# santiagolmedo/gnn_qot_estimation

Measured on NVIDIA B200. Metric: lightpath_infer_graphs_per_sec, higher is better.
Workload: dtype f32

## Files before the change

### gnn_qot_estimation_b200/csrc/lightpath_stream.cu

```cuda
#include <algorithm>
#include <type_traits>

#include "lightpath_common.cuh"

namespace qot {

constexpr int kTG = 16;
constexpr int kTNodes = 704;
constexpr int kTEdges = 2688;
constexpr int kTMaxE = 248;
#ifndef QOT_ST_WARPS
#define QOT_ST_WARPS 15
#endif
#ifndef QOT_ST_XSTAGES
#define QOT_ST_XSTAGES 7
#endif
#ifndef QOT_ST_DSTAGES
#define QOT_ST_DSTAGES 4
#endif
#ifndef QOT_STH_WARPS
#define QOT_STH_WARPS 14
#endif
#ifndef QOT_STH_XSTAGES
#define QOT_STH_XSTAGES 6
#endif
#ifndef QOT_STH_DSTAGES
#define QOT_STH_DSTAGES 3
#endif
template <bool kHead> struct StCfg;
template <> struct StCfg<false> {
  static constexpr int kX = QOT_ST_XSTAGES;
  static constexpr int kD = QOT_ST_DSTAGES;
  static constexpr int kConsumers = QOT_ST_WARPS;
  static constexpr int kThreads = 32 * (1 + kConsumers);
};
template <> struct StCfg<true> {
  static constexpr int kX = QOT_STH_XSTAGES;
  static constexpr int kD = QOT_STH_DSTAGES;
  static constexpr int kConsumers = QOT_STH_WARPS;
  static constexpr int kThreads = 32 * (8 + kConsumers - 2);
};
constexpr int kStGroupWarps = 4;
constexpr int kStXBytes = kTNodes * kF * 4;
constexpr int kStDBytes = kTEdges * 8;

struct alignas(16) StTileInfo {
  qot_lp_batch_t d;
  int64_t g0;
  int64_t nb0, eb0;
  int xn, en;
  unsigned xlead, dlead;
  int ng;
  int pad;
};
static_assert(sizeof(qot_lp_batch_t) == 128, "the descriptor is copied as eight 16-byte pieces");

struct alignas(128) StStage {
  alignas(128) unsigned char xs[kStXBytes + 16];
  alignas(16) long long ptrs[3][kTG + 2];
  StTileInfo info;
};
struct alignas(128) StDStage {
  alignas(128) unsigned char ds[kStDBytes + 16];
};

struct StGenericArgs {
  const float* x;
  const int64_t* esrc;
  const int64_t* edst;
  float* z;
  float* out;
  int64_t* lut_batch;
  int32_t* lut_node;
  int32_t* status;
  int64_t N, E, g0;
  int64_t p[4][6];
};

struct StWarpScratch {
  StGenericArgs gargs;
  int msg[4][kSubMsg];
  int raw[4][kSubMsg];
};

constexpr int kZPitch = 21;
constexpr int kGroupTiles = 8;
struct StHeadSmem {
  alignas(1024) float b2[2][4][32 * 32];
  float zrow[2][128 * kZPitch];
  float* optr[2][128];
  alignas(8) unsigned long long zfull[2];
  alignas(8) unsigned long long zfree[2];
  alignas(8) unsigned long long aready;
  alignas(8) unsigned long long dready;
  unsigned tmem_base;
  alignas(16) float wf[kHC * kF];
  alignas(16) float shift[kHC];
  alignas(16) float b1[kHid];
  alignas(16) float w2[QOT_OUT * kHid];
  float bo[4];
};
struct StNoHead {};

template <bool kHead>
struct StSmemT {
  typename std::conditional<kHead, StHeadSmem, StNoHead>::type head;
  StDStage dstage[StCfg<kHead>::kD];
  StStage stage[StCfg<kHead>::kX];
  float4 asp[8][6];
  float4 adp[4][kF];
  StWarpScratch wsc[StCfg<kHead>::kConsumers];
  float gen[256];
  alignas(8) unsigned long long full[StCfg<kHead>::kX];
  alignas(8) unsigned long long empty[StCfg<kHead>::kX];
  alignas(8) unsigned long long dempty[StCfg<kHead>::kD];
  int next_unit;
  int gen_lock;
};
extern __shared__ __align__(1024) char st_smem_raw[];
template <bool kHead>
__device__ __forceinline__ StSmemT<kHead>& st_smem() {
  const unsigned off = (1024u - (static_cast<unsigned>(__cvta_generic_to_shared(st_smem_raw)) & 1023u)) & 1023u;
  return *reinterpret_cast<StSmemT<kHead>*>(st_smem_raw + off);
}
static_assert(sizeof(StSmemT<false>) + 1024 <= 227 * 1024, "lp_stream_kernel: shared memory over the 227 KB block limit");
static_assert(sizeof(StSmemT<true>) + 1024 <= 227 * 1024, "lp_stream_kernel<head>: shared memory over the 227 KB block limit");

#ifdef QOT_ST_TRACE
__device__ unsigned long long* g_st_trace = nullptr;
#define ST_DECL() long long st_acc_[8] = {0, 0, 0, 0, 0, 0, 0, 0}
#define ST_T0() const long long st_t0_ = clock64()
#define ST_T1() const long long st_t1_ = clock64()
#define ST_PARAM , long long* st_acc_
#define ST_ARG , st_acc_
#define ST_ACC1(slot) do { st_acc_[slot] += clock64() - st_t1_; } while (0)
#define ST_ACC(slot) do { st_acc_[slot] += clock64() - st_t0_; } while (0)
#define ST_FLUSH() do { if (g_st_trace && lane == 0) for (int i_ = 0; i_ < 8; ++i_) if (st_acc_[i_]) atomicAdd(g_st_trace + blockIdx.x * 8 + i_, static_cast<unsigned long long>(st_acc_[i_])); } while (0)
#else
#define ST_DECL() do {} while (0)
#define ST_T0() do {} while (0)
#define ST_T1() do {} while (0)
#define ST_PARAM
#define ST_ARG
#define ST_ACC1(slot) do {} while (0)
#define ST_ACC(slot) do {} while (0)
#define ST_FLUSH() do {} while (0)
#endif
__device__ __forceinline__ unsigned st_smem_u32(const void* p) { return static_cast<unsigned>(__cvta_generic_to_shared(p)); }
#ifndef QOT_ST_SUSPEND_NS
#define QOT_ST_SUSPEND_NS 20000
#endif
__device__ __forceinline__ bool st_try_wait(unsigned bar, unsigned parity) {
  unsigned ok;
  asm volatile(
      "{ .reg .pred p; mbarrier.try_wait.parity.shared::cta.b64 p, [%1], %2, %3; selp.u32 %0, 1, 0, p; }"
      : "=r"(ok) : "r"(bar), "r"(parity), "r"(QOT_ST_SUSPEND_NS) : "memory");
  return ok != 0u;
}
template <unsigned kSleepNs = 40>
__device__ __forceinline__ bool st_wait(unsigned bar, unsigned parity) {
  if (st_try_wait(bar, parity)) return true;
  unsigned long long t0;
  asm volatile("mov.u64 %0, %%globaltimer;" : "=l"(t0));
  for (;;) {
#pragma unroll 1
    for (int i = 0; i < 256; ++i) {
      __nanosleep(kSleepNs);
      if (st_try_wait(bar, parity)) return true;
    }
    unsigned long long t1;
    asm volatile("mov.u64 %0, %%globaltimer;" : "=l"(t1));
    if (t1 - t0 > 2000000000ull) return false;
  }
}
__device__ __forceinline__ void st_arrive(unsigned bar) {
  asm volatile("mbarrier.arrive.shared::cta.b64 _, [%0];" ::"r"(bar) : "memory");
}
__device__ __forceinline__ void st_mbar_init(unsigned long long* bar, int count) {
  asm volatile("mbarrier.init.shared::cta.b64 [%0], %1;" ::"r"(st_smem_u32(bar)), "r"(count) : "memory");
}

template <bool kHead>
__device__ __noinline__ void st_producer(const qot_lp_batch_t* __restrict__ bt, int nb, int64_t tpb,
                                         int64_t tile_base, int64_t total_tiles, int lane) {
  StSmemT<kHead>& sm = st_smem<kHead>();
  const int64_t G = gridDim.x;
  const int64_t my_tiles = (total_tiles - blockIdx.x + G - 1) / G;
  ST_DECL();
  for (int64_t kb = 0; kb < my_tiles; kb += 32) {
    int b = 0;
    long long g0 = 0, nb0 = 0, nb1 = 0, eb0 = 0, eb1 = 0, dN = 0, dE = 0, dB = 0;
    const float* dx = nullptr;
    const int64_t *dei = nullptr, *dptr = nullptr, *deptr = nullptr, *dlptr = nullptr;
    if (kb + lane < my_tiles) {
      const int64_t T = tile_base + blockIdx.x + (kb + lane) * G;
      b = st_batch_of(bt, nb, tpb, tile_base, T);
      const qot_lp_batch_t& d = bt[b];
      dx = d.x; dei = d.edge_index; dptr = d.ptr; deptr = d.edge_ptr; dlptr = d.lut_ptr;
      dN = d.N; dE = d.E; dB = d.B;
      g0 = (T - d.tile0) * kTG;
      const int64_t gE = min(static_cast<int64_t>(g0 + kTG), static_cast<int64_t>(dB));
      nb0 = dptr[g0]; nb1 = dptr[gE];
      eb0 = deptr[g0]; eb1 = deptr[gE];
    }
    const int cnt = static_cast<int>(min(static_cast<int64_t>(32), my_tiles - kb));
    for (int j = 0; j < cnt; ++j) {
      const int64_t k = kb + j;
      constexpr int kStStages = StCfg<kHead>::kX, kStDStages = StCfg<kHead>::kD;
      const int s = static_cast<int>(k % kStStages);
      const unsigned ph = static_cast<unsigned>((k / kStStages) & 1);
      StStage& st = sm.stage[s];
      const int sd_ = static_cast<int>(k % kStDStages);
      StDStage& dst_stage = sm.dstage[sd_];
      const unsigned fbar = st_smem_u32(&sm.full[s]);
      {
        ST_T0();
        st_wait(st_smem_u32(&sm.empty[s]), ph ^ 1u);
        st_wait(st_smem_u32(&sm.dempty[sd_]), static_cast<unsigned>((k / kStDStages) & 1) ^ 1u);
        ST_ACC(0);
      }
      ST_T0();
      const int tb = __shfl_sync(kFull, b, j);
      const long long tg0 = __shfl_sync(kFull, g0, j), tB = __shfl_sync(kFull, dB, j);
      const int64_t* tptr = reinterpret_cast<const int64_t*>(__shfl_sync(kFull, reinterpret_cast<unsigned long long>(dptr), j));
      const int64_t* teptr = reinterpret_cast<const int64_t*>(__shfl_sync(kFull, reinterpret_cast<unsigned long long>(deptr), j));
      const int64_t* tlptr = reinterpret_cast<const int64_t*>(__shfl_sync(kFull, reinterpret_cast<unsigned long long>(dlptr), j));
#pragma unroll
      for (int r = 0; r < 2; ++r) {
        const int idx = lane + 32 * r;
        if (idx < 3 * (kTG + 1)) {
          const int which = idx / (kTG + 1), i = idx % (kTG + 1);
          const int64_t gi = min(static_cast<int64_t>(tg0 + i), static_cast<int64_t>(tB));
          const int64_t* src = (which == 0 ? tptr : which == 1 ? teptr : tlptr) + gi;
          asm volatile("cp.async.ca.shared.global [%0], [%1], 8;" ::"r"(st_smem_u32(&st.ptrs[which][i])), "l"(src) : "memory");
        }
      }
      if (lane >= 24)
        asm volatile("cp.async.cg.shared.global [%0], [%1], 16;"
                     ::"r"(st_smem_u32(reinterpret_cast<char*>(&st.info.d) + 16 * (lane - 24))),
                       "l"(reinterpret_cast<const char*>(bt + tb) + 16 * (lane - 24)) : "memory");
      asm volatile("cp.async.mbarrier.arrive.noinc.shared::cta.b64 [%0];" ::"r"(fbar) : "memory");
      if (lane == j) {
        int xn = 0, en = 0;
        if (nb0 >= 0 && nb1 >= nb0 && nb1 <= dN && nb1 - nb0 <= kTNodes) xn = static_cast<int>(nb1 - nb0);
        if (eb0 >= 0 && eb1 >= eb0 && eb1 <= dE && eb1 - eb0 <= kTEdges) en = static_cast<int>(eb1 - eb0);
        if (xn == 0 || (en == 0 && eb1 != eb0)) { xn = 0; en = 0; }
        const int64_t* edst = dei + dE;
        const uintptr_t xa = reinterpret_cast<uintptr_t>(dx) + static_cast<uintptr_t>(xn > 0 ? nb0 : 0) * (kF * 4);
        const uintptr_t da = reinterpret_cast<uintptr_t>(edst) + static_cast<uintptr_t>(en > 0 ? eb0 : 0) * 8;
        const unsigned xlead = static_cast<unsigned>(xa & 15), dlead = static_cast<unsigned>(da & 15);
        const uintptr_t xs0 = xa - xlead, ds0 = da - dlead;
        const unsigned xspan = xlead + static_cast<unsigned>(xn) * (kF * 4), dspan = dlead + static_cast<unsigned>(en) * 8;
        unsigned xbytes = (xspan + 15u) & ~15u, dbytes = (dspan + 15u) & ~15u;
        if (xs0 + xbytes > reinterpret_cast<uintptr_t>(dx) + static_cast<uintptr_t>(dN) * (kF * 4)) xbytes = xspan & ~15u;
        if (ds0 + dbytes > reinterpret_cast<uintptr_t>(edst) + static_cast<uintptr_t>(dE) * 8) dbytes = dspan & ~15u;
        if (xn == 0) xbytes = 0;
        if (en == 0) dbytes = 0;
        if (xn > 0)
          for (unsigned o = xbytes; o < xspan; o += 4)
            *reinterpret_cast<float*>(st.xs + o) = *reinterpret_cast<const float*>(xs0 + o);
        if (en > 0 && dspan > dbytes)
          *reinterpret_cast<long long*>(dst_stage.ds + dbytes) = *reinterpret_cast<const long long*>(ds0 + dbytes);
        StTileInfo& ti = st.info;
        ti.g0 = g0; ti.nb0 = nb0; ti.eb0 = eb0;
        ti.xn = xn; ti.en = en; ti.xlead = xlead; ti.dlead = dlead;
        ti.ng = static_cast<int>(min(static_cast<int64_t>(kTG), static_cast<int64_t>(dB - g0)));
        asm volatile("mbarrier.arrive.expect_tx.shared::cta.b64 _, [%0], %1;" ::"r"(fbar), "r"(xbytes + dbytes) : "memory");
        if (xbytes)
          asm volatile("cp.async.bulk.shared::cluster.global.mbarrier::complete_tx::bytes [%0], [%1], %2, [%3];"
                       ::"r"(st_smem_u32(st.xs)), "l"(xs0), "r"(xbytes), "r"(fbar) : "memory");
        if (dbytes)
          asm volatile("cp.async.bulk.shared::cluster.global.mbarrier::complete_tx::bytes [%0], [%1], %2, [%3];"
                       ::"r"(st_smem_u32(dst_stage.ds)), "l"(ds0), "r"(dbytes), "r"(fbar) : "memory");
      }
      __syncwarp();
      ST_ACC(1);
    }
  }
  ST_FLUSH();
}

template <bool kHead>
__device__ __noinline__ void st_generic(int cw, unsigned todo, const float* __restrict__ prep, int lut_col, int lane) {
  StSmemT<kHead>& sm = st_smem<kHead>();
  const StGenericArgs& ga = sm.wsc[cw].gargs;
  float* scratch = sm.gen;
  int* lock = &sm.gen_lock;
  const float* gx = ga.x;
  const int64_t N = ga.N;
  if (lane == 0)
    while (atomicCAS(lock, 0, 1) != 0) __nanosleep(200);
  __syncwarp();
  float* s_y = scratch;
  float* s_z = scratch + 128;
  int* s_m = reinterpret_cast<int*>(scratch + 160);
#pragma unroll 1
  for (int s = 0; s < 4; ++s) {
    if (!((todo >> s) & 1u)) continue;
    const int64_t gn0 = ga.p[s][0], gn1 = ga.p[s][1], ge0 = ga.p[s][2], ge1 = ga.p[s][3], gl0 = ga.p[s][4], gl1 = ga.p[s][5];
    int64_t orow = gl0;
    int found = 0;
    if (gn0 >= 0 && gn1 <= N && ge0 >= 0 && ge1 <= ga.E) {
      for (int64_t nbq = gn0; nbq < gn1; nbq += 32) {
        const int64_t node = nbq + lane;
        unsigned mask = __ballot_sync(kFull, node < gn1 && gx[node * kF + lut_col] == 1.0f);
        while (mask) {
          const int bit = __ffs(mask) - 1;
          mask &= mask - 1;
          ++found;
          if (orow < gl1) {
            const int64_t i = nbq + bit;
            if constexpr (kHead) {
              const float ov = lut_row_global<true>(XRaw{gx}, ga.esrc, ga.edst, ge0, ge1, N, i, prep, prep + kOffWf, s_m, s_z, s_y, lane);
              if (lane < QOT_OUT) ga.out[orow * QOT_OUT + lane] = ov;
            } else {
              lut_row_global<false>(XRaw{gx}, ga.esrc, ga.edst, ge0, ge1, N, i, prep, nullptr, s_m, s_z, nullptr, lane);
              if (lane < kHeads * kF) ga.z[orow * (kHeads * kF) + lane] = s_z[(lane / kF) * 8 + lane % kF];
            }
            if (lane == 0) {
              ga.lut_batch[orow] = ga.g0 + s;
              ga.lut_node[orow] = static_cast<int32_t>(i);
            }
            __syncwarp();
            ++orow;
          }
        }
      }
    }
    if (lane == 0 && found != gl1 - gl0) atomicOr(ga.status, 1);
  }
  __syncwarp();
  if (lane == 0) {
    __threadfence_block();
    atomicExch(lock, 0);
  }
}

template <bool kHead, bool kSym>
__device__ __forceinline__ void st_consume_tile(int k, int cw, const float* __restrict__ prep, int lut_col, int gw,
                                                int lane ST_PARAM) {
  StSmemT<kHead>& sm = st_smem<kHead>();
  StWarpScratch& gs = sm.wsc[cw];
  StStage& st = sm.stage[k % StCfg<kHead>::kX];
  const StDStage& dstg = sm.dstage[k % StCfg<kHead>::kD];
  const unsigned ebar = st_smem_u32(&sm.empty[k % StCfg<kHead>::kX]), dbar = st_smem_u32(&sm.dempty[k % StCfg<kHead>::kD]);
  const float4 (*__restrict__ asp)[6] = sm.asp;
  const int sg = lane >> 3, sl = lane & 7;
  const int gl = gw * 4 + sg;
  const StTileInfo& ti = st.info;
  int n = 0, ne = 0, xoff = 0, eoff = 0, lrows = 0;
  bool active, fits;
  {
    const int64_t n0 = st.ptrs[0][gl], n1 = st.ptrs[0][gl + 1];
    const int64_t e0 = st.ptrs[1][gl], e1 = st.ptrs[1][gl + 1];
    const int64_t l0 = st.ptrs[2][gl], l1 = st.ptrs[2][gl + 1];
    const int64_t nb0 = ti.nb0, eb0 = ti.eb0;
    const int xn = ti.xn, en = ti.en;
    active = gl < ti.ng;
    fits = active && xn > 0 && n1 >= n0 && e1 >= e0 && (n1 - n0) <= kMaxN && (e1 - e0) <= kTMaxE &&
           n0 >= nb0 && (n1 - nb0) <= xn && e0 >= eb0 && (e1 - eb0) <= en && l1 >= l0 && (l1 - l0) <= kMaxN;
    if (fits) {
      n = static_cast<int>(n1 - n0); ne = static_cast<int>(e1 - e0);
      xoff = static_cast<int>(n0 - nb0); eoff = static_cast<int>(e0 - eb0);
      lrows = static_cast<int>(l1 - l0);
    }
    if (active && ti.g0 + gl == ti.d.B - 1 && sl == 0) ti.d.n_lut[0] = static_cast<int32_t>(l1);
  }
  const float* sx = reinterpret_cast<const float*>(st.xs + ti.xlead) + xoff * kF;
  const long long* sd = reinterpret_cast<const long long*>(dstg.ds + ti.dlead) + eoff;
  const int hx = sl >> 1;
  const bool odd = (sl & 1) != 0;

  int cnt = 0, il = -1;
  {
    unsigned m = 0u;
    const int rmax = (__reduce_max_sync(kFull, n) + 7) >> 3;
#pragma unroll
    for (int r = 0; r < kMaxN / 8; ++r) {
      if (r < rmax) {
        const int node = sl + 8 * r;
        if (node < n && sx[node * kF + lut_col] == 1.0f) m |= 1u << r;
      }
    }
    cnt = __popc(m);
    int first = m ? 8 * (__ffs(m) - 1) + sl : 0x7fff;
#pragma unroll
    for (int o = 1; o <= 4; o <<= 1) {
      cnt += __shfl_xor_sync(kFull, cnt, o);
      first = min(first, __shfl_xor_sync(kFull, first, o));
    }
    if (cnt) il = first;
  }
  bool ok = fits && cnt == 1 && lrows == 1;
  if (fits && sl == 0 && cnt != lrows) atomicOr(ti.d.status, 1);

  int* msg = gs.msg[sg];
  int mc = 0;
  if constexpr (kSym) {
    const int c = ((ne + 7) >> 3) | 1;
    const int eb = sl * c;
    const int tmax = ok ? min(c, ne - eb) : 0;
    const int cmax = __reduce_max_sync(kFull, tmax);
    const int target = static_cast<int>(st.ptrs[0][gl]) + il;
    const int* sde = reinterpret_cast<const int*>(sd + eb);
    unsigned em[4] = {0u, 0u, 0u, 0u}, lm[4] = {0u, 0u, 0u, 0u};
#pragma unroll
    for (int t4 = 0; t4 < 32; t4 += 4) {
      if (t4 < cmax) {
#pragma unroll
        for (int i = 0; i < 4; ++i) {
          const int t = t4 + i;
          if (t < 31) {
            const int d = sde[2 * t];
            asm("{ .reg .pred p, q;\n\t"
                "setp.eq.s32 p, %2, %3;\n\t"
                "setp.lt.s32 q, %2, %3;\n\t"
                "@p or.b32 %0, %0, %4;\n\t"
                "@q or.b32 %1, %1, %4; }"
                : "+r"(em[i]), "+r"(lm[i]) : "r"(d), "r"(target), "r"(1u << t));
          }
        }
      }
    }
    const unsigned vm = (1u << max(tmax, 0)) - 1u;
    int pack = __popc((em[0] | em[1] | em[2] | em[3]) & vm) | (__popc((lm[0] | lm[1] | lm[2] | lm[3]) & vm) << 16);
#pragma unroll
    for (int o = 1; o <= 4; o <<= 1) pack += __shfl_xor_sync(kFull, pack, o);
    const int deg = pack & 0xffff, start = pack >> 16;
    if (deg > kSubMsg - 1) ok = false;
    int* raw = gs.raw[sg];
    int v0 = 0x7fffffff, v1 = 0x7fffffff;
    bool bad = false;
    if (ok) {
      const int n0i = target - il;
      if (sl < deg) {
        const int w = static_cast<int>(sd[start + sl]) - n0i;
        bad |= w < 0 || w >= n;
        if (w != il) v0 = w;
      }
      if (sl + 8 < deg) {
        const int w = static_cast<int>(sd[start + sl + 8]) - n0i;
        bad |= w < 0 || w >= n;
        if (w != il) v1 = w;
      }
    }
    raw[sl] = v0;
    raw[sl + 8] = v1;
    if (((__ballot_sync(kFull, bad) >> (8 * sg)) & 0xffu) != 0u) ok = false;
    const int dmax = __reduce_max_sync(kFull, ok ? deg : 0);
    __syncwarp();
    if (lane == 0) st_arrive(dbar);
    int r0 = 0, r1 = 0;
    for (int j = 0; j < dmax; ++j) {
      const int w = raw[j];
      r0 += w < v0;
      r1 += w < v1;
    }
    const bool k0 = ok && v0 != 0x7fffffff, k1 = ok && v1 != 0x7fffffff;
    if (k0) msg[r0] = v0;
    if (k1) msg[r1] = v1;
    const unsigned kb0 = (__ballot_sync(kFull, k0) >> (8 * sg)) & 0xffu, kb1 = (__ballot_sync(kFull, k1) >> (8 * sg)) & 0xffu;
    mc = __popc(kb0) + __popc(kb1);
  } else {
    {
      const int c = ((ne + 7) >> 3) | 1;
      const int eb = sl * c;
      const int tmax = ok ? min(c, ne - eb) : 0;
      const int cmax = __reduce_max_sync(kFull, tmax);
      const long long target = st.ptrs[0][gl] + il;
      const int tlo = static_cast<int>(target), thi = static_cast<int>(target >> 32);
      const int2* sde = reinterpret_cast<const int2*>(sd + eb);
      unsigned hm = 0u;
#pragma unroll
      for (int t4 = 0; t4 < 32; t4 += 4) {
        if (t4 < cmax) {
#pragma unroll
          for (int i = 0; i < 4; ++i) {
            const int t = t4 + i;
            if (t < 31) {
              const int2 d = sde[t];
              asm("{ .reg .pred p;\n\t"
                  "setp.eq.s32 p, %1, %3;\n\t"
                  "setp.eq.and.s32 p, %2, %4, p;\n\t"
                  "@p or.b32 %0, %0, %5; }"
                  : "+r"(hm) : "r"(d.x), "r"(d.y), "r"(tlo), "r"(thi), "r"(1u << t));
            }
          }
        }
      }
      hm &= (1u << max(tmax, 0)) - 1u;
      const int h = __popc(hm);
      int incl = h;
#pragma unroll
      for (int o = 1; o <= 4; o <<= 1) {
        const int up = __shfl_up_sync(kFull, incl, o, 8);
        if (sl >= o) incl += up;
      }
      mc = __shfl_sync(kFull, incl, (lane & ~7) + 7);
      int pos = incl - h;
      while (hm) {
        const int t = __ffs(hm) - 1;
        hm &= hm - 1u;
        if (pos < kSubMsg - 1) msg[pos] = eb + t;
        ++pos;
      }
    }
    if (mc > kSubMsg - 1) ok = false;
    __syncwarp();
    if (lane == 0) st_arrive(dbar);
    {
      int kept = 0;
      bool outside = false;
      const int64_t* __restrict__ esrc = ti.d.edge_index + st.ptrs[1][gl];
      const int64_t n0 = st.ptrs[0][gl], N = ti.d.N;
#pragma unroll
      for (int t0 = 0; t0 < kSubMsg; t0 += 8) {
        if (__any_sync(kFull, ok && t0 < mc)) {
          const int t = t0 + sl;
          long long sj = -1;
          if (ok && t < mc) sj = esrc[msg[t]];
          const bool inN = static_cast<uint64_t>(sj) < static_cast<uint64_t>(N);
          const long long sloc = sj - n0;
          const bool inslab = sloc >= 0 && sloc < n;
          const bool keep = inslab && sloc != il;
          outside |= ((__ballot_sync(kFull, inN && !inslab) >> (8 * sg)) & 0xffu) != 0u;
          const unsigned sub = (__ballot_sync(kFull, keep) >> (8 * sg)) & 0xffu;
          __syncwarp();
          if (keep) msg[kept + __popc(sub & ((1u << sl) - 1u))] = static_cast<int>(sloc);
          kept += __popc(sub);
          __syncwarp();
        }
      }
      if (outside) ok = false;
      mc = kept;
    }
  }
  if (ok && sl == 0) msg[mc] = il;
  ++mc;
  __syncwarp();

  {
    float d[kHeads];
    const int ils = ok ? il : 0;
#pragma unroll
    for (int i = 0; i < kHeads; ++i) d[i] = 0.f;
#pragma unroll
    for (int k = 0; k < kF; ++k) {
      const float xi = sx[ils * kF + k];
      const float4 b = sm.adp[hx][k];
      d[0] = fmaf(xi, b.x, d[0]); d[1] = fmaf(xi, b.y, d[1]);
      d[2] = fmaf(xi, b.z, d[2]); d[3] = fmaf(xi, b.w, d[3]);
    }
    float mx[kHeads], acc3[3] = {0.f, 0.f, 0.f};
#pragma unroll
    for (int i = 0; i < kHeads; ++i) mx[i] = -INFINITY;
    const int o0 = odd ? 3 : 0;
#pragma unroll
    for (int r0 = 0; r0 < kSubMsg; r0 += 8) {
      if (__any_sync(kFull, ok && r0 < mc)) {
        const bool valid = ok && r0 + sl < mc;
        const float* xr = sx + (valid ? msg[r0 + sl] : 0) * kF;
        float q[6];
        const float x2 = xr[2];
        q[0] = xr[o0]; q[1] = xr[o0 + 1]; q[3] = xr[3 - o0]; q[4] = xr[4 - o0];
        q[2] = odd ? 1.0f : x2;
        q[5] = odd ? x2 : 1.0f;
        float a[kHeads], mr[kHeads], m2[kHeads];
#pragma unroll
        for (int i = 0; i < kHeads; ++i) a[i] = d[i];
#pragma unroll
        for (int m = 0; m < 6; ++m) {
          const float4 w = asp[sl][m];
          a[0] = fmaf(q[m], w.x, a[0]); a[1] = fmaf(q[m], w.y, a[1]);
          a[2] = fmaf(q[m], w.z, a[2]); a[3] = fmaf(q[m], w.w, a[3]);
        }
#pragma unroll
        for (int i = 0; i < kHeads; ++i) {
          const float t = a[i] > 0.f ? a[i] : 0.2f * a[i];
          a[i] = valid ? t : -INFINITY;
        }
#pragma unroll
        for (int i = 0; i < kHeads; ++i) mr[i] = fmaxf(a[i], __shfl_xor_sync(kFull, a[i], 1));
#pragma unroll
        for (int i = 0; i < kHeads; ++i) m2[i] = fmaxf(mr[i], __shfl_xor_sync(kFull, mr[i ^ 1], 2));
#pragma unroll
        for (int i = 0; i < kHeads; ++i) mr[i] = fmaxf(m2[i], __shfl_xor_sync(kFull, m2[i ^ 2], 4));
        float v[24];
        float scarg = 0.f;
#pragma unroll
        for (int i = 0; i < kHeads; ++i) {
          const float mn = fmaxf(fmaxf(mx[i], mr[i]), -1e30f);
          const float p = valid ? expf(a[i] - mn) : 0.f;
// ... 180 lines not shown
        float4 acc = sh4[h * 8 + c4];
#pragma unroll
        for (int f = 0; f < kF; ++f) {
          const float4 w = wf4[(h * kF + f) * 8 + c4];
          const float zf = z[h * kF + f];
          acc.x = fmaf(zf, w.x, acc.x); acc.y = fmaf(zf, w.y, acc.y);
          acc.z = fmaf(zf, w.z, acc.z); acc.w = fmaf(zf, w.w, acc.w);
        }
        const float y[4] = {fmaxf(acc.x, 0.f), fmaxf(acc.y, 0.f), fmaxf(acc.z, 0.f), fmaxf(acc.w, 0.f)};
#pragma unroll
        for (int j = 0; j < 4; ++j) {
          const unsigned hb = __float_as_uint(y[j]) & 0xffffe000u;
          hi[c4 * 4 + j] = hb;
          lo[c4 * 4 + j] = __float_as_uint(y[j] - __uint_as_float(hb)) + 0x1000u;
        }
      }
      st_tmem_st32(tb + static_cast<unsigned>(h * 32), hi);
      st_tmem_st32(tb + kTmemALo + static_cast<unsigned>(h * 32), lo);
    }
    asm volatile("tcgen05.wait::st.sync.aligned;" ::: "memory");
    asm volatile("tcgen05.fence::before_thread_sync;" ::: "memory");
    __syncwarp();
    if (lane == 0) st_arrive(st_smem_u32(&hs.aready));
    {
      ST_T1();
      if (!st_wait<100>(st_smem_u32(&hs.dready), static_cast<unsigned>(g & 1))) break;
      ST_ACC1(6);
    }
    asm volatile("tcgen05.fence::after_thread_sync;" ::: "memory");
    unsigned r[32];
    {
      unsigned r1[32], r2[32];
      st_tmem_ld32(tb + kTmemD, r);
      st_tmem_ld32(tb + kTmemD + 32u, r1);
      st_tmem_ld32(tb + kTmemD + 64u, r2);
#pragma unroll
      for (int j = 0; j < 32; ++j)
        r[j] = __float_as_uint((__uint_as_float(r[j]) + __uint_as_float(r1[j])) + __uint_as_float(r2[j]));
      st_tmem_ld32(tb + kTmemD + 96u, r1);
      st_tmem_ld32(tb + kTmemD + 128u, r2);
#pragma unroll
      for (int j = 0; j < 32; ++j)
        r[j] = __float_as_uint((__uint_as_float(r[j]) + __uint_as_float(r1[j])) + __uint_as_float(r2[j]));
    }
    float o3[QOT_OUT];
#pragma unroll
    for (int k = 0; k < QOT_OUT; ++k) o3[k] = hs.bo[k];
#pragma unroll
    for (int j4 = 0; j4 < 8; ++j4) {
      const float4 b1 = reinterpret_cast<const float4*>(hs.b1)[j4];
      float hv[4] = {__uint_as_float(r[4 * j4]) + b1.x, __uint_as_float(r[4 * j4 + 1]) + b1.y,
                     __uint_as_float(r[4 * j4 + 2]) + b1.z, __uint_as_float(r[4 * j4 + 3]) + b1.w};
#pragma unroll
      for (int j = 0; j < 4; ++j) hv[j] = hv[j] > 0.f ? hv[j] : 0.01f * hv[j];
#pragma unroll
      for (int k = 0; k < QOT_OUT; ++k) {
        const float4 w2 = reinterpret_cast<const float4*>(hs.w2 + k * kHid)[j4];
        o3[k] = fmaf(hv[0], w2.x, o3[k]); o3[k] = fmaf(hv[1], w2.y, o3[k]);
        o3[k] = fmaf(hv[2], w2.z, o3[k]); o3[k] = fmaf(hv[3], w2.w, o3[k]);
      }
    }
    if (op) {
      op[0] = o3[0]; op[1] = o3[1]; op[2] = o3[2];
    }
    asm volatile("tcgen05.fence::before_thread_sync;" ::: "memory");
  }
  ST_ACC(7);
  ST_FLUSH();
}

template <bool kHead, bool kSym>
__global__ void __launch_bounds__(StCfg<kHead>::kThreads, 1)
lp_stream_kernel(const qot_lp_batch_t* __restrict__ batches, int n_batches, int64_t tiles_per_batch,
                 int64_t total_tiles, const float* __restrict__ prep, int lut_col) {
  StSmemT<kHead>& sm = st_smem<kHead>();
  const int tid = threadIdx.x, lane = tid & 31, warp = tid >> 5;
  const int my_tiles = static_cast<int>((total_tiles - blockIdx.x + gridDim.x - 1) / gridDim.x);
  const int ngroups = (my_tiles + kGroupTiles - 1) / kGroupTiles;
  if (tid == 0) {
    for (int s = 0; s < StCfg<kHead>::kX; ++s) {
      st_mbar_init(&sm.full[s], 33);
      st_mbar_init(&sm.empty[s], kStGroupWarps);
    }
    for (int s = 0; s < StCfg<kHead>::kD; ++s) st_mbar_init(&sm.dempty[s], kStGroupWarps);
    if constexpr (kHead) {
      for (int i = 0; i < 2; ++i) {
        st_mbar_init(&sm.head.zfull[i], kGroupTiles * kStGroupWarps);
        st_mbar_init(&sm.head.zfree[i], 4);
      }
      st_mbar_init(&sm.head.aready, 4);
      st_mbar_init(&sm.head.dready, 1);
    }
    asm volatile("fence.mbarrier_init.release.cluster;" ::: "memory");
    sm.next_unit = 0;
    sm.gen_lock = 0;
  }
  if (tid < 48) (&sm.asp[0][0])[tid] = __ldg(reinterpret_cast<const float4*>(prep + kOffAsP) + tid);
  if (tid >= 64 && tid < 64 + 4 * kF) (&sm.adp[0][0])[tid - 64] = __ldg(reinterpret_cast<const float4*>(prep + kOffAdP) + tid - 64);
  if constexpr (kHead) {
    float4* b2 = reinterpret_cast<float4*>(&sm.head.b2[0][0][0]);
    for (int i = tid; i < kB2swFloats / 4; i += StCfg<kHead>::kThreads)
      b2[i] = __ldg(reinterpret_cast<const float4*>(prep + kOffB2sw) + i);
    for (int i = tid; i < kHC * kF; i += StCfg<kHead>::kThreads) sm.head.wf[i] = __ldg(prep + kOffWf + i);
    if (tid < kHC) sm.head.shift[tid] = __ldg(prep + kOffShift + tid);
    if (tid < kHid) sm.head.b1[tid] = __ldg(prep + kOffB1 + tid);
    if (tid < QOT_OUT * kHid) sm.head.w2[tid] = __ldg(prep + kOffW2 + tid);
    if (tid < QOT_OUT) sm.head.bo[tid] = __ldg(prep + kOffB2 + tid);
    if (warp == 4) {
      asm volatile("tcgen05.alloc.cta_group::1.sync.aligned.shared::cta.b32 [%0], %1;" ::"r"(st_smem_u32(&sm.head.tmem_base)),
                   "r"(kTmemCols)
                   : "memory");
      asm volatile("tcgen05.relinquish_alloc_permit.cta_group::1.sync.aligned;" ::: "memory");
    }
    asm volatile("fence.proxy.async.shared::cta;" ::: "memory");
    asm volatile("tcgen05.fence::before_thread_sync;" ::: "memory");
  }
  __syncthreads();
  if constexpr (kHead) asm volatile("tcgen05.fence::after_thread_sync;" ::: "memory");
  if (warp == 0) {
    st_producer<kHead>(batches, n_batches, tiles_per_batch, batches[0].tile0, total_tiles, lane);
    return;
  }
  int cw = warp - 1;
  if constexpr (kHead) {
    if (warp == 1) {
      st_head_mma(ngroups, lane);
      return;
    }
    if (warp >= 4 && warp < 8) {
      st_head_epilogue(my_tiles, ngroups, warp - 4, lane);
      asm volatile("tcgen05.fence::before_thread_sync;" ::: "memory");
      asm volatile("bar.sync 1, 128;" ::: "memory");
      if (warp == 4)
        asm volatile("tcgen05.dealloc.cta_group::1.sync.aligned.b32 %0, %1;" ::"r"(sm.head.tmem_base), "r"(kTmemCols) : "memory");
      return;
    }
    cw = warp < 4 ? warp - 2 : warp - 6;
  }
  const int tiles_padded = kHead ? ngroups * kGroupTiles : my_tiles;
  ST_DECL();
  for (;;) {
    int u = 0;
    if (lane == 0) u = atomicAdd(&sm.next_unit, 1);
    u = __shfl_sync(kFull, u, 0);
    const int k = u >> 2, gw = u & 3;
    if (k >= tiles_padded) break;
    if constexpr (kHead) {
      if (k >= my_tiles) {
        const int grp = k / kGroupTiles, buf = grp & 1;
        if (!st_wait(st_smem_u32(&sm.head.zfree[buf]), static_cast<unsigned>((grp >> 1) & 1) ^ 1u)) break;
        if (lane < 4) sm.head.optr[buf][(k % kGroupTiles) * kTG + gw * 4 + lane] = nullptr;
        __syncwarp();
        if (lane == 0) st_arrive(st_smem_u32(&sm.head.zfull[buf]));
        continue;
      }
    }
    const int s = k % StCfg<kHead>::kX;
    const unsigned ph = static_cast<unsigned>((k / StCfg<kHead>::kX) & 1);
    {
      ST_T0();
      if (!st_wait(st_smem_u32(&sm.full[s]), ph)) {
        if (lane == 0) atomicOr(batches[0].status, 4);
        break;
      }
      ST_ACC(2);
    }
    ST_T0();
// ... 207 lines not shown
```

Baseline: 1.230 billion.

## Read edge destinations from L2 via prefetch instead of staging them in shared memory

Removes the shared-memory ring of edge-destination stages, along with its dempty barriers and bulk copies. Destination indices are now brought into L2 with cp.async.bulk.prefetch a few tiles ahead, and consumers read them directly from global memory with vectorized non-allocating loads in an interleaved pair layout. The freed shared memory lets the head variant use more x stages (6 to 10). The cost is extra global/L2 load latency in the consumer scan, more complex index bookkeeping for the interleaved layout, and reliance on the prefetched lines still being resident in L2 when consumers read them.

Result: slower. 1.032 billion, median of 6 (-16.1%).

```diff
diff --git a/gnn_qot_estimation_b200/csrc/lightpath_stream.cu b/gnn_qot_estimation_b200/csrc/lightpath_stream.cu
--- a/gnn_qot_estimation_b200/csrc/lightpath_stream.cu
+++ b/gnn_qot_estimation_b200/csrc/lightpath_stream.cu
@@ -15,43 +15,38 @@
 #ifndef QOT_ST_XSTAGES
 #define QOT_ST_XSTAGES 7
 #endif
-#ifndef QOT_ST_DSTAGES
-#define QOT_ST_DSTAGES 4
-#endif
 #ifndef QOT_STH_WARPS
 #define QOT_STH_WARPS 14
 #endif
 #ifndef QOT_STH_XSTAGES
-#define QOT_STH_XSTAGES 6
+#define QOT_STH_XSTAGES 10
 #endif
-#ifndef QOT_STH_DSTAGES
-#define QOT_STH_DSTAGES 3
+#ifndef QOT_ST_DPREFETCH
+#define QOT_ST_DPREFETCH 4
 #endif
+constexpr int kStDPrefetch = QOT_ST_DPREFETCH;
+static_assert(kStDPrefetch >= 0 && kStDPrefetch < 32, "the prefetch distance must stay inside one 32-tile look-ahead");
 template <bool kHead> struct StCfg;
 template <> struct StCfg<false> {
   static constexpr int kX = QOT_ST_XSTAGES;
-  static constexpr int kD = QOT_ST_DSTAGES;
   static constexpr int kConsumers = QOT_ST_WARPS;
   static constexpr int kThreads = 32 * (1 + kConsumers);
 };
 template <> struct StCfg<true> {
   static constexpr int kX = QOT_STH_XSTAGES;
-  static constexpr int kD = QOT_STH_DSTAGES;
   static constexpr int kConsumers = QOT_STH_WARPS;
   static constexpr int kThreads = 32 * (8 + kConsumers - 2);
 };
 constexpr int kStGroupWarps = 4;
 constexpr int kStXBytes = kTNodes * kF * 4;
-constexpr int kStDBytes = kTEdges * 8;
 
 struct alignas(16) StTileInfo {
   qot_lp_batch_t d;
   int64_t g0;
   int64_t nb0, eb0;
   int xn, en;
-  unsigned xlead, dlead;
+  unsigned xlead;
   int ng;
-  int pad;
 };
 static_assert(sizeof(qot_lp_batch_t) == 128, "the descriptor is copied as eight 16-byte pieces");
 
@@ -59,9 +54,6 @@
   alignas(128) unsigned char xs[kStXBytes + 16];
   alignas(16) long long ptrs[3][kTG + 2];
   StTileInfo info;
-};
-struct alignas(128) StDStage {
-  alignas(128) unsigned char ds[kStDBytes + 16];
 };
 
 struct StGenericArgs {
@@ -105,7 +97,6 @@
 template <bool kHead>
 struct StSmemT {
   typename std::conditional<kHead, StHeadSmem, StNoHead>::type head;
-  StDStage dstage[StCfg<kHead>::kD];
   StStage stage[StCfg<kHead>::kX];
   float4 asp[8][6];
   float4 adp[4][kF];
@@ -113,7 +104,6 @@
   float gen[256];
   alignas(8) unsigned long long full[StCfg<kHead>::kX];
   alignas(8) unsigned long long empty[StCfg<kHead>::kX];
-  alignas(8) unsigned long long dempty[StCfg<kHead>::kD];
   int next_unit;
   int gen_lock;
 };
@@ -203,20 +193,32 @@
       nb0 = dptr[g0]; nb1 = dptr[gE];
       eb0 = deptr[g0]; eb1 = deptr[gE];
     }
+    int xn = 0, en = 0;
+    if (nb0 >= 0 && nb1 >= nb0 && nb1 <= dN && nb1 - nb0 <= kTNodes) xn = static_cast<int>(nb1 - nb0);
+    if (eb0 >= 0 && eb1 >= eb0 && eb1 <= dE && eb1 - eb0 <= kTEdges) en = static_cast<int>(eb1 - eb0);
+    if (xn == 0 || (en == 0 && eb1 != eb0)) { xn = 0; en = 0; }
+    auto prefetch_dst = [&]() {
+      if (en == 0) return;
+      const uintptr_t edst = reinterpret_cast<uintptr_t>(dei + dE);
+      const uintptr_t da = edst + static_cast<uintptr_t>(eb0) * 8, ds0 = da & ~static_cast<uintptr_t>(15);
+      const unsigned dspan = static_cast<unsigned>(da - ds0) + static_cast<unsigned>(en) * 8;
+      unsigned dbytes = (dspan + 15u) & ~15u;
+      if (ds0 + dbytes > edst + static_cast<uintptr_t>(dE) * 8) dbytes = dspan & ~15u;
+      if (dbytes) asm volatile("cp.async.bulk.prefetch.L2.global [%0], %1;" ::"l"(ds0), "r"(dbytes) : "memory");
+    };
     const int cnt = static_cast<int>(min(static_cast<int64_t>(32), my_tiles - kb));
+    if (lane < kStDPrefetch && lane < cnt) prefetch_dst();
     for (int j = 0; j < cnt; ++j) {
       const int64_t k = kb + j;
-      constexpr int kStStages = StCfg<kHead>::kX, kStDStages = StCfg<kHead>::kD;
+      constexpr int kStStages = StCfg<kHead>::kX;
       const int s = static_cast<int>(k % kStStages);
       const unsigned ph = static_cast<unsigned>((k / kStStages) & 1);
       StStage& st = sm.stage[s];
-      const int sd_ = static_cast<int>(k % kStDStages);
-      StDStage& dst_stage = sm.dstage[sd_];
       const unsigned fbar = st_smem_u32(&sm.full[s]);
+      if (kStDPrefetch > 0 && lane == j + kStDPrefetch && lane < cnt) prefetch_dst();
       {
         ST_T0();
         st_wait(st_smem_u32(&sm.empty[s]), ph ^ 1u);
-        st_wait(st_smem_u32(&sm.dempty[sd_]), static_cast<unsigned>((k / kStDStages) & 1) ^ 1u);
         ST_ACC(0);
       }
       ST_T0();
@@ -241,37 +243,24 @@
                        "l"(reinterpret_cast<const char*>(bt + tb) + 16 * (lane - 24)) : "memory");
       asm volatile("cp.async.mbarrier.arrive.noinc.shared::cta.b64 [%0];" ::"r"(fbar) : "memory");
       if (lane == j) {
-        int xn = 0, en = 0;
-        if (nb0 >= 0 && nb1 >= nb0 && nb1 <= dN && nb1 - nb0 <= kTNodes) xn = static_cast<int>(nb1 - nb0);
-        if (eb0 >= 0 && eb1 >= eb0 && eb1 <= dE && eb1 - eb0 <= kTEdges) en = static_cast<int>(eb1 - eb0);
-        if (xn == 0 || (en == 0 && eb1 != eb0)) { xn = 0; en = 0; }
-        const int64_t* edst = dei + dE;
         const uintptr_t xa = reinterpret_cast<uintptr_t>(dx) + static_cast<uintptr_t>(xn > 0 ? nb0 : 0) * (kF * 4);
-        const uintptr_t da = reinterpret_cast<uintptr_t>(edst) + static_cast<uintptr_t>(en > 0 ? eb0 : 0) * 8;
-        const unsigned xlead = static_cast<unsigned>(xa & 15), dlead = static_cast<unsigned>(da & 15);
-        const uintptr_t xs0 = xa - xlead, ds0 = da - dlead;
-        const unsigned xspan = xlead + static_cast<unsigned>(xn) * (kF * 4), dspan = dlead + static_cast<unsigned>(en) * 8;
-        unsigned xbytes = (xspan + 15u) & ~15u, dbytes = (dspan + 15u) & ~15u;
+        const unsigned xlead = static_cast<unsigned>(xa & 15);
+        const uintptr_t xs0 = xa - xlead;
+        const unsigned xspan = xlead + static_cast<unsigned>(xn) * (kF * 4);
+        unsigned xbytes = (xspan + 15u) & ~15u;
         if (xs0 + xbytes > reinterpret_cast<uintptr_t>(dx) + static_cast<uintptr_t>(dN) * (kF * 4)) xbytes = xspan & ~15u;
-        if (ds0 + dbytes > reinterpret_cast<uintptr_t>(edst) + static_cast<uintptr_t>(dE) * 8) dbytes = dspan & ~15u;
         if (xn == 0) xbytes = 0;
-        if (en == 0) dbytes = 0;
         if (xn > 0)
           for (unsigned o = xbytes; o < xspan; o += 4)
             *reinterpret_cast<float*>(st.xs + o) = *reinterpret_cast<const float*>(xs0 + o);
-        if (en > 0 && dspan > dbytes)
-          *reinterpret_cast<long long*>(dst_stage.ds + dbytes) = *reinterpret_cast<const long long*>(ds0 + dbytes);
         StTileInfo& ti = st.info;
         ti.g0 = g0; ti.nb0 = nb0; ti.eb0 = eb0;
-        ti.xn = xn; ti.en = en; ti.xlead = xlead; ti.dlead = dlead;
+        ti.xn = xn; ti.en = en; ti.xlead = xlead;
         ti.ng = static_cast<int>(min(static_cast<int64_t>(kTG), static_cast<int64_t>(dB - g0)));
-        asm volatile("mbarrier.arrive.expect_tx.shared::cta.b64 _, [%0], %1;" ::"r"(fbar), "r"(xbytes + dbytes) : "memory");
+        asm volatile("mbarrier.arrive.expect_tx.shared::cta.b64 _, [%0], %1;" ::"r"(fbar), "r"(xbytes) : "memory");
         if (xbytes)
           asm volatile("cp.async.bulk.shared::cluster.global.mbarrier::complete_tx::bytes [%0], [%1], %2, [%3];"
                        ::"r"(st_smem_u32(st.xs)), "l"(xs0), "r"(xbytes), "r"(fbar) : "memory");
-        if (dbytes)
-          asm volatile("cp.async.bulk.shared::cluster.global.mbarrier::complete_tx::bytes [%0], [%1], %2, [%3];"
-                       ::"r"(st_smem_u32(dst_stage.ds)), "l"(ds0), "r"(dbytes), "r"(fbar) : "memory");
       }
       __syncwarp();
       ST_ACC(1);
@@ -336,19 +325,73 @@
   }
 }
 
+#ifndef QOT_ST_SCAN_CHUNK
+#define QOT_ST_SCAN_CHUNK 4
+#endif
+constexpr int kStScanChunk = QOT_ST_SCAN_CHUNK;
+struct StDstPairs {
+  const char* base;
+  int jlo, jn;
+  int lead;
+  unsigned valid;
+  unsigned fix;
+};
+__device__ __forceinline__ unsigned st_lowmask(int n) { return n >= 32 ? ~0u : (1u << n) - 1u; }
+__device__ __forceinline__ StDstPairs st_dst_pairs(const long long* gd, int64_t ge0, int ne, int64_t E, int sl, bool ok) {
+  StDstPairs q;
+  q.lead = static_cast<int>((reinterpret_cast<uintptr_t>(gd) >> 3) & 1u);
+  q.base = reinterpret_cast<const char*>(gd) - 8 * q.lead;
+  const int np = (ne + q.lead + 1) >> 1;
+  const int plo = (q.lead && ge0 == 0) ? 1 : 0;
+  const int phi = ge0 - q.lead + 2 * static_cast<int64_t>(np) <= E ? np : np - 1;
+  const int r = ne + q.lead - 2 * sl;
+  const int nv = !ok || r <= 0 ? 0 : min(32, 2 * (r >> 4) + min(r & 15, 2));
+  q.valid = st_lowmask(nv) & ~((sl == 0 && q.lead) ? 1u : 0u);
+  q.jlo = sl < plo ? 1 : 0;
+  q.jn = ok && phi > sl ? (phi - sl + 7) >> 3 : 0;
+  q.fix = q.valid & ~(st_lowmask(2 * q.jn) & ~st_lowmask(2 * q.jlo));
+  return q;
+}
+__device__ __forceinline__ int4 st_ld_l2_v4(const char* p) {
+  int4 v;
+  asm volatile("ld.global.nc.L1::no_allocate.v4.s32 {%0, %1, %2, %3}, [%4];"
+               : "=r"(v.x), "=r"(v.y), "=r"(v.z), "=r"(v.w) : "l"(p));
+  return v;
+}
+__device__ __forceinline__ long long st_ld_l2_b64(const void* p) {
+  long long v;
+  asm volatile("ld.global.nc.L1::no_allocate.s64 %0, [%1];" : "=l"(v) : "l"(p));
+  return v;
+}
+__device__ __forceinline__ void st_count_dst(unsigned& em, unsigned& lm, int d, int target, unsigned bit) {
+  asm("{ .reg .pred p, q;\n\t"
+      "setp.eq.s32 p, %2, %3;\n\t"
+      "setp.lt.s32 q, %2, %3;\n\t"
+      "@p or.b32 %0, %0, %4;\n\t"
+      "@q or.b32 %1, %1, %4; }"
+      : "+r"(em), "+r"(lm) : "r"(d), "r"(target), "r"(bit));
+}
+__device__ __forceinline__ void st_match_dst(unsigned& hm, int dlo, int dhi, int tlo, int thi, unsigned bit) {
+  asm("{ .reg .pred p;\n\t"
+      "setp.eq.s32 p, %1, %3;\n\t"
+      "setp.eq.and.s32 p, %2, %4, p;\n\t"
+      "@p or.b32 %0, %0, %5; }"
+      : "+r"(hm) : "r"(dlo), "r"(dhi), "r"(tlo), "r"(thi), "r"(bit));
+}
+
 template <bool kHead, bool kSym>
 __device__ __forceinline__ void st_consume_tile(int k, int cw, const float* __restrict__ prep, int lut_col, int gw,
                                                 int lane ST_PARAM) {
   StSmemT<kHead>& sm = st_smem<kHead>();
   StWarpScratch& gs = sm.wsc[cw];
   StStage& st = sm.stage[k % StCfg<kHead>::kX];
-  const StDStage& dstg = sm.dstage[k % StCfg<kHead>::kD];
-  const unsigned ebar = st_smem_u32(&sm.empty[k % StCfg<kHead>::kX]), dbar = st_smem_u32(&sm.dempty[k % StCfg<kHead>::kD]);
+  const unsigned ebar = st_smem_u32(&sm.empty[k % StCfg<kHead>::kX]);
   const float4 (*__restrict__ asp)[6] = sm.asp;
   const int sg = lane >> 3, sl = lane & 7;
   const int gl = gw * 4 + sg;
   const StTileInfo& ti = st.info;
-  int n = 0, ne = 0, xoff = 0, eoff = 0, lrows = 0;
+  int n = 0, ne = 0, xoff = 0, lrows = 0;
+  int64_t ge0 = 0;
   bool active, fits;
   {
     const int64_t n0 = st.ptrs[0][gl], n1 = st.ptrs[0][gl + 1];
@@ -361,13 +404,15 @@
            n0 >= nb0 && (n1 - nb0) <= xn && e0 >= eb0 && (e1 - eb0) <= en && l1 >= l0 && (l1 - l0) <= kMaxN;
     if (fits) {
       n = static_cast<int>(n1 - n0); ne = static_cast<int>(e1 - e0);
-      xoff = static_cast<int>(n0 - nb0); eoff = static_cast<int>(e0 - eb0);
+      xoff = static_cast<int>(n0 - nb0);
+      ge0 = e0;
       lrows = static_cast<int>(l1 - l0);
     }
     if (active && ti.g0 + gl == ti.d.B - 1 && sl == 0) ti.d.n_lut[0] = static_cast<int32_t>(l1);
   }
   const float* sx = reinterpret_cast<const float*>(st.xs + ti.xlead) + xoff * kF;
-  const long long* sd = reinterpret_cast<const long long*>(dstg.ds + ti.dlead) + eoff;
+  const int64_t E = ti.d.E;
+  const long long* gd = reinterpret_cast<const long long*>(ti.d.edge_index) + E + ge0;
   const int hx = sl >> 1;
   const bool odd = (sl & 1) != 0;
 
@@ -397,32 +442,36 @@
   int* msg = gs.msg[sg];
   int mc = 0;
   if constexpr (kSym) {
-    const int c = ((ne + 7) >> 3) | 1;
-    const int eb = sl * c;
-    const int tmax = ok ? min(c, ne - eb) : 0;
-    const int cmax = __reduce_max_sync(kFull, tmax);
+    const StDstPairs q = st_dst_pairs(gd, ge0, ne, E, sl, ok);
+    const int cmax = __reduce_max_sync(kFull, q.jn);
     const int target = static_cast<int>(st.ptrs[0][gl]) + il;
-    const int* sde = reinterpret_cast<const int*>(sd + eb);
-    unsigned em[4] = {0u, 0u, 0u, 0u}, lm[4] = {0u, 0u, 0u, 0u};
-#pragma unroll
-    for (int t4 = 0; t4 < 32; t4 += 4) {
-      if (t4 < cmax) {
-#pragma unroll
-        for (int i = 0; i < 4; ++i) {
-          const int t = t4 + i;
-          if (t < 31) {
-            const int d = sde[2 * t];
-            asm("{ .reg .pred p, q;\n\t"
-                "setp.eq.s32 p, %2, %3;\n\t"
-                "setp.lt.s32 q, %2, %3;\n\t"
-                "@p or.b32 %0, %0, %4;\n\t"
-                "@q or.b32 %1, %1, %4; }"
-                : "+r"(em[i]), "+r"(lm[i]) : "r"(d), "r"(target), "r"(1u << t));
-          }
-        }
-      }
-    }
-    const unsigned vm = (1u << max(tmax, 0)) - 1u;
+    unsigned em[4] = {0u, 0u, 0u, 0u}, lm[4] = {0u, 0u, 0u, 0u}, hi = 0u;
+#pragma unroll
+    for (int j0 = 0; j0 < 16; j0 += kStScanChunk) {
+      if (j0 < cmax) {
+        int4 v[kStScanChunk];
+#pragma unroll
+        for (int i = 0; i < kStScanChunk; ++i) {
+          const int j = j0 + i;
+          v[i] = make_int4(0x7fffffff, 0, 0x7fffffff, 0);
+          if (j >= q.jlo && j < q.jn) v[i] = st_ld_l2_v4(q.base + 16 * (sl + 8 * j));
+        }
+#pragma unroll
+        for (int i = 0; i < kStScanChunk; ++i) {
+          const int b = 2 * (j0 + i);
+          st_count_dst(em[b & 3], lm[b & 3], v[i].x, target, 1u << b);
+          st_count_dst(em[(b + 1) & 3], lm[(b + 1) & 3], v[i].z, target, 2u << b);
+          hi |= static_cast<unsigned>(v[i].y | v[i].w);
+        }
+      }
+    }
+    for (unsigned f = q.fix; f; f &= f - 1u) {
+      const int b = __ffs(f) - 1;
+      const long long d = st_ld_l2_b64(q.base + 16 * (sl + 8 * (b >> 1)) + 8 * (b & 1));
+      st_count_dst(em[0], lm[0], static_cast<int>(d), target, 1u << b);
+      hi |= static_cast<unsigned>(d >> 32);
+    }
+    const unsigned vm = q.valid;
     int pack = __popc((em[0] | em[1] | em[2] | em[3]) & vm) | (__popc((lm[0] | lm[1] | lm[2] | lm[3]) & vm) << 16);
 #pragma unroll
     for (int o = 1; o <= 4; o <<= 1) pack += __shfl_xor_sync(kFull, pack, o);
@@ -430,16 +479,16 @@
     if (deg > kSubMsg - 1) ok = false;
     int* raw = gs.raw[sg];
     int v0 = 0x7fffffff, v1 = 0x7fffffff;
-    bool bad = false;
+    bool bad = hi != 0u;
     if (ok) {
       const int n0i = target - il;
       if (sl < deg) {
-        const int w = static_cast<int>(sd[start + sl]) - n0i;
+        const int w = static_cast<int>(st_ld_l2_b64(gd + start + sl)) - n0i;
         bad |= w < 0 || w >= n;
         if (w != il) v0 = w;
       }
       if (sl + 8 < deg) {
-        const int w = static_cast<int>(sd[start + sl + 8]) - n0i;
+        const int w = static_cast<int>(st_ld_l2_b64(gd + start + sl + 8)) - n0i;
         bad |= w < 0 || w >= n;
         if (w != il) v1 = w;
       }
@@ -449,7 +498,6 @@
     if (((__ballot_sync(kFull, bad) >> (8 * sg)) & 0xffu) != 0u) ok = false;
     const int dmax = __reduce_max_sync(kFull, ok ? deg : 0);
     __syncwarp();
-    if (lane == 0) st_arrive(dbar);
     int r0 = 0, r1 = 0;
     for (int j = 0; j < dmax; ++j) {
       const int w = raw[j];
@@ -463,51 +511,52 @@
     mc = __popc(kb0) + __popc(kb1);
   } else {
     {
-      const int c = ((ne + 7) >> 3) | 1;
-      const int eb = sl * c;
-      const int tmax = ok ? min(c, ne - eb) : 0;
-      const int cmax = __reduce_max_sync(kFull, tmax);
+      const StDstPairs q = st_dst_pairs(gd, ge0, ne, E, sl, ok);
+      const int cmax = __reduce_max_sync(kFull, q.jn);
       const long long target = st.ptrs[0][gl] + il;
       const int tlo = static_cast<int>(target), thi = static_cast<int>(target >> 32);
-      const int2* sde = reinterpret_cast<const int2*>(sd + eb);
       unsigned hm = 0u;
 #pragma unroll
-      for (int t4 = 0; t4 < 32; t4 += 4) {
-        if (t4 < cmax) {
-#pragma unroll
-          for (int i = 0; i < 4; ++i) {
-            const int t = t4 + i;
-            if (t < 31) {
-              const int2 d = sde[t];
-              asm("{ .reg .pred p;\n\t"
-                  "setp.eq.s32 p, %1, %3;\n\t"
-                  "setp.eq.and.s32 p, %2, %4, p;\n\t"
-                  "@p or.b32 %0, %0, %5; }"
-                  : "+r"(hm) : "r"(d.x), "r"(d.y), "r"(tlo), "r"(thi), "r"(1u << t));
-            }
+      for (int j0 = 0; j0 < 16; j0 += kStScanChunk) {
+        if (j0 < cmax) {
+          int4 v[kStScanChunk];
+#pragma unroll
+          for (int i = 0; i < kStScanChunk; ++i) {
+            const int j = j0 + i;
+            v[i] = make_int4(-1, -1, -1, -1);
+            if (j >= q.jlo && j < q.jn) v[i] = st_ld_l2_v4(q.base + 16 * (sl + 8 * j));
           }
-        }
-      }
-      hm &= (1u << max(tmax, 0)) - 1u;
-      const int h = __popc(hm);
-      int incl = h;
-#pragma unroll
-      for (int o = 1; o <= 4; o <<= 1) {
-        const int up = __shfl_up_sync(kFull, incl, o, 8);
-        if (sl >= o) incl += up;
-      }
-      mc = __shfl_sync(kFull, incl, (lane & ~7) + 7);
-      int pos = incl - h;
-      while (hm) {
-        const int t = __ffs(hm) - 1;
-        hm &= hm - 1u;
-        if (pos < kSubMsg - 1) msg[pos] = eb + t;
-        ++pos;
+#pragma unroll
+          for (int i = 0; i < kStScanChunk; ++i) {
+            const int b = 2 * (j0 + i);
+            st_match_dst(hm, v[i].x, v[i].y, tlo, thi, 1u << b);
+            st_match_dst(hm, v[i].z, v[i].w, tlo, thi, 2u << b);
+          }
+        }
+      }
+      for (unsigned f = q.fix; f; f &= f - 1u) {
+        const int b = __ffs(f) - 1;
+        const long long d = st_ld_l2_b64(q.base + 16 * (sl + 8 * (b >> 1)) + 8 * (b & 1));
+        st_match_dst(hm, static_cast<int>(d), static_cast<int>(d >> 32), tlo, thi, 1u << b);
+      }
+      hm &= q.valid;
+      unsigned ho[8];
+#pragma unroll
+      for (int l = 0; l < 8; ++l) ho[l] = __shfl_sync(kFull, hm, (lane & ~7) + l);
+      mc = 0;
+#pragma unroll
+      for (int l = 0; l < 8; ++l) mc += __popc(ho[l]);
+      for (unsigned f = hm; f; f &= f - 1u) {
+        const int b = __ffs(f) - 1, j2 = b & ~1;
+        int pos = __popc(hm & st_lowmask(b));
+#pragma unroll
+        for (int l = 0; l < 8; ++l)
+          if (l != sl) pos += __popc(ho[l] & st_lowmask(l < sl ? j2 + 2 : j2));
+        if (pos < kSubMsg - 1) msg[pos] = 16 * (b >> 1) + 2 * sl + (b & 1) - q.lead;
       }
     }
     if (mc > kSubMsg - 1) ok = false;
     __syncwarp();
-    if (lane == 0) st_arrive(dbar);
     {
       int kept = 0;
       bool outside = false;
@@ -854,7 +903,6 @@
       st_mbar_init(&sm.full[s], 33);
       st_mbar_init(&sm.empty[s], kStGroupWarps);
     }
-    for (int s = 0; s < StCfg<kHead>::kD; ++s) st_mbar_init(&sm.dempty[s], kStGroupWarps);
     if constexpr (kHead) {
       for (int i = 0; i < 2; ++i) {
         st_mbar_init(&sm.head.zfull[i], kGroupTiles * kStGroupWarps);
```
